# epam/Zstandard

Hardware: AMD Instinct MI355X
Metric: GiB/s compress @ level 3, 64 KiB chunks (higher is better)
Workload: dtype u8; 1 GPU; 4096 independent 65536 B chunks per GPU per step, level 3, BASELINE config[1] shape (Silesia unavailable offline -> Zipf-token log stream, SURVEY 8d); chunks_per_gpu=4096, chunk_bytes=65536, level=3, parallelism=chunks sharded over 1 GPU(s), no collective in the data path

## Files before the change

zstandard_amd/csrc/dict_train.hip:

```cpp
#include <hipcub/hipcub.hpp>
#include "zsmi_wave.h"
#include "entropy_kernels.hip"
#include "zsmi_fse.h"
#include "zsmi_status.h"
#include "zsmi_ctx.h"
#include <algorithm>

static const uint32_t kTrainDefaultF = 20, kTrainMinF = 12, kTrainMaxF = 26;
static const uint32_t kTrainDictSizeMin = 256, kTrainContentMin = 128;
static const uint32_t kTrainMaxZeroRun = 10;
static const uint32_t kTrainThreads = 1024, kTrainPerThread = 8;

struct ZsTrainCand { uint32_t k, d, pad0, pad1; uint32_t *freq; uint8_t *content; };

__device__ __forceinline__ uint32_t train_hash(const uint8_t *p, uint32_t d, uint32_t f)
{
    const uint64_t v = zs_load64(p);
    if (d == 6) return (uint32_t)(((v << 16) * 227718039650203ull) >> (64 - f));
    return (uint32_t)((v * 0xCF1BBCDCB7A56463ull) >> (64 - f));
}

__global__ void k_train_freq(const uint8_t *__restrict__ samples, uint32_t nbDmers, uint32_t d, uint32_t f, const uint64_t *__restrict__ ends, uint32_t nTrain,
                             uint2 *__restrict__ info, uint64_t *__restrict__ keys, uint32_t *__restrict__ freq)
{
// ... 112 lines not shown
        const uint32_t segSize = min(ne - nb + d - 1, tail);
        __syncthreads();
        if (segSize < d) break;
        tail -= segSize;
        for (uint32_t i = tid; i < segSize; i += kTrainThreads) content[tail + i] = samples[nb + i];
        __syncthreads();
    }
    if (tid == 0) tails[blockIdx.x] = tail;
}

__global__ void __launch_bounds__(64) k_train_id(const uint8_t *__restrict__ content, uint32_t size, uint32_t given, uint32_t *__restrict__ id)
{
    const uint64_t h = xxh64_quad<16>(content, size);
    if (threadIdx.x == 0) *id = given ? given : (uint32_t)(h % 2147450880ull) + 32768u;
}

__device__ static uint32_t train_scaled(const uint32_t *raw, uint32_t n, uint32_t *out, uint64_t limit)
{
    uint64_t total = 0;
    for (uint32_t s = 0; s < n; s++) total += (uint64_t)raw[s] + 1;
    uint32_t shift = 0;
    while ((total >> shift) >= limit) shift++;
    uint32_t sum = 0;
    for (uint32_t s = 0; s < n; s++) { out[s] = max(1u, (uint32_t)(((uint64_t)raw[s] + 1) >> shift)); sum += out[s]; }
    return sum;
}

__global__ void __launch_bounds__(256) k_train_tables(const uint32_t *__restrict__ stats, const uint8_t *__restrict__ content, uint32_t contentSize, uint32_t cap,
                                                      const uint32_t *__restrict__ dictID, uint8_t *__restrict__ hdr, uint8_t *__restrict__ out, uint32_t *__restrict__ result)
{
    __shared__ K3Lds L;
    __shared__ uint32_t cnt[64], misc[4];
    __shared__ int16_t norm[64];
    const uint32_t tid = threadIdx.x, wave = tid >> 6, lane = tid & 63u;
    const uint32_t hcap = 1024;
    if (tid == 0) { misc[0] = 0; misc[1] = 0; train_scaled(stats, 256, L.count, 1u << 23); }
    __syncthreads();
    const uint32_t lit = L.count[tid];
    for (uint32_t maxBits = ZS_HUF_MAXBITS; maxBits >= 8; maxBits--) {
        L.count[tid] = lit;
        __syncthreads();
        const uint32_t tableLog = huffLengths(L, 255, maxBits);
        huffCodesAndWeights(L, 255, tableLog);
        if (wave == 0) { const uint32_t hs = writeHuffHeaderWave(L, hdr + 8, 256, 255, tableLog); if (lane == 0) misc[0] = hs; }
        __syncthreads();
        if (misc[0]) break;
        __syncthreads();
    }
    if (wave == 0 && misc[0]) {
        uint32_t pos = 8 + misc[0];
        const uint32_t ofMax = zs_highbit(contentSize + (128u << 10));
        const uint32_t maxes[3] = { min(ofMax, (uint32_t)MaxOff), MaxML, MaxLL }, logs[3] = { OffFSELog, MLFSELog, LLFSELog }, base[3] = { 320, 384, 256 };
        bool ok = true;
        uint32_t &scaledTotal = L.misc[0], &ncountBytes = L.misc[1];
        for (uint32_t t = 0; t < 3 && ok; t++) {
            if (lane == 0) scaledTotal = train_scaled(stats + base[t], maxes[t] + 1, cnt, 1u << 30);
            wave_sync();
            normalizeCountsWave(norm, logs[t], cnt, scaledTotal, maxes[t]);
            if (lane == 0) ncountBytes = writeNCount(hdr + pos, hcap - pos, norm, maxes[t], logs[t]);
            wave_sync();
            const uint32_t w = ncountBytes;
            ok = w != 0; pos += w;
        }
        ok = ok && pos + 12 <= hcap;
        if (lane == 0) {
            const uint32_t id = *dictID, words[5] = { 0xEC30A437u, id, 1u, 4u, 8u };
            for (uint32_t i = 0; i < 2; i++) zs_store32(hdr + 4 * i, words[i]);
            if (ok) for (uint32_t i = 0; i < 3; i++) zs_store32(hdr + pos + 4 * i, words[2 + i]);
            pos += 12;
            misc[1] = (ok && pos <= hcap && pos < cap) ? pos : 0u;
        }
    }
    __syncthreads();
    const uint32_t hs = misc[1];
    if (!hs) { if (tid == 0) *result = 0; return; }
    const uint32_t keep = min(contentSize, cap - hs);
    for (uint32_t i = tid; i < hs; i += 256) out[i] = hdr[i];
    zs_block_copy(out + hs, content + (contentSize - keep), keep, tid, 256);
    if (tid == 0) *result = hs + keep;
}

__global__ void k_train_gather(const uint8_t *__restrict__ src, const uint64_t *__restrict__ offs , const uint32_t *__restrict__ sizes,
                               uint32_t n, uint8_t *__restrict__ dst)
{
    const uint32_t i = blockIdx.x;
    zs_block_copy(dst + offs[n + i], src + offs[i], sizes[i], threadIdx.x, blockDim.x);
}

extern "C" unsigned zsmi_getDictID(const void *dict, size_t dictSize)
{
    const uint8_t *d = (const uint8_t *)dict;
    if (!d || dictSize < 8 || rd32(d) != 0xEC30A437u) return 0;
    return rd32(d + 4);
}

namespace {
struct TrainPlan {
    uint32_t f = kTrainDefaultF, steps = 40;
    int level = 3;
    double split = 0.75;
    std::vector<std::pair<uint32_t, uint32_t>> cands;
    bool search = false;
};
}

static int trainParams(const zsmi_fastCoverParams *p, size_t cap, uint64_t total, uint32_t nb, TrainPlan &t)
{
    if (cap < kTrainDictSizeMin) return ZSMI_error_dstSize_tooSmall;
    if (!p) return ZSMI_error_GENERIC;
    if (p->d != 0 && p->d != 6 && p->d != 8) return ZSMI_error_parameter_outOfBound;
    if (p->f != 0 && (p->f < kTrainMinF || p->f > kTrainMaxF)) return ZSMI_error_parameter_outOfBound;
    if (p->accel > 1) return ZSMI_error_parameter_outOfBound;
    if (!(p->splitPoint == 0.0 || (p->splitPoint > 0.0 && p->splitPoint <= 1.0))) return ZSMI_error_parameter_outOfBound;
    if (p->k != 0 && (p->k < (p->d ? p->d : 8u) || p->k > cap || p->k > 65536u)) return ZSMI_error_parameter_outOfBound;
// ... 233 lines not shown
```

zstandard_amd/csrc/entropy_kernels.hip:

```cpp
#ifndef ZSMI_ENTROPY_KERNELS_HIP
#define ZSMI_ENTROPY_KERNELS_HIP
#include "zsmi_device.h"
#include "zsmi_status.h"
#include "zsmi_scratch.h"
#include "zsmi_wave.h"
#include "zsmi_fse.h"
#ifdef ZSMI_DEBUG_HOOKS
#define ZS_STOP_AT(v) (stopAt == (v))
#define ZS_STOPPED (stopAt != 0)
#else
#define ZS_STOP_AT(v) false
#define ZS_STOPPED false
#endif

__device__ __forceinline__ uint32_t llCodeOf(uint32_t ll)
{
    uint32_t c = zs_highbit(ll | 1u) + 19;
    c = (ll < 64) ? 24u : c;
    c = (ll < 48) ? 22u + ((ll - 32) >> 3) : c;
    c = (ll < 32) ? 20u + ((ll - 24) >> 2) : c;
    c = (ll < 24) ? 16u + ((ll - 16) >> 1) : c;
    return (ll < 16) ? ll : c;
}
__device__ __forceinline__ uint32_t mlCodeOf(uint32_t x)
{
    uint32_t c = zs_highbit(x | 1u) + 36;
    c = (x < 128) ? 42u : c;
    c = (x < 96) ? 40u + ((x - 64) >> 4) : c;
    c = (x < 64) ? 38u + ((x - 48) >> 3) : c;
    c = (x < 48) ? 36u + ((x - 40) >> 2) : c;
    c = (x < 40) ? 32u + ((x - 32) >> 1) : c;
    return (x < 32) ? x : c;
}
__device__ __forceinline__ uint32_t llExtraOf(uint32_t ll, uint32_t &bits)
{
    const uint32_t h = zs_highbit(ll | 1u);
    uint32_t v = ll - (1u << h), b = h;
    if (ll < 64) { v = ll - 48; b = 4; }
    if (ll < 48) { v = ll & 7u; b = 3; }
    if (ll < 32) { v = ll & 3u; b = 2; }
    if (ll < 24) { v = ll & 1u; b = 1; }
    if (ll < 16) { v = 0; b = 0; }
    bits = b; return v;
}
__device__ __forceinline__ uint32_t mlExtraOf(uint32_t x, uint32_t &bits)
{
    const uint32_t h = zs_highbit(x | 1u);
    uint32_t v = x - (1u << h), b = h;
    if (x < 128) { v = x - 96; b = 5; }
    if (x < 96) { v = x & 15u; b = 4; }
    if (x < 64) { v = x & 7u; b = 3; }
    if (x < 48) { v = x & 3u; b = 2; }
    if (x < 40) { v = x & 1u; b = 1; }
    if (x < 32) { v = 0; b = 0; }
    bits = b; return v;
}

struct FseCT {
    uint16_t stateTable[512];
    int32_t  deltaFindState[64];
    uint32_t deltaNbBits[64];
    uint32_t tableLog;
    uint32_t rle;
};
#define ZS_COST_NONE 0xFFFFu
struct ZsCDictTables {
    FseCT ct[3];
    uint16_t cost[3][64];
    uint32_t hufCodeNb[256];
    uint32_t hufLog;
};
__device__ __forceinline__ uint32_t fseSymbolCost(uint32_t nv, uint32_t tableLog)
{
    nv = max(nv, 1u);
    const uint32_t maxBitsOut = nv > 1 ? tableLog - zs_highbit(nv - 1) : tableLog;
    return maxBitsOut * 256u - ((((nv << maxBitsOut) - (1u << tableLog)) << 8) >> tableLog);
}
#ifndef ZS_LIT_MINWG
#define ZS_LIT_MINWG 8
#endif
struct K3Lds {
    uint32_t count[256];
    uint8_t  nbBits[256];
    uint32_t codeNb[256];
    uint32_t leafW[256];
    uint16_t leafSym[256];
    uint8_t  lenOfRank[256];
    uint8_t  weights[256];
    union {
        struct { uint32_t pkg[10][256]; uint32_t S[512]; uint32_t npk[12]; } pm;
        struct { FseCT ct; FseBuild build; uint16_t stepOut[256]; uint32_t bits[64]; } fse;
        struct { FseCT ct; FseBuild build; } cd[3];
        uint32_t tile[4][208];
        uint32_t hist[8][257];
        struct { uint32_t T[2052]; uint32_t wpar[4], wcnt[4]; uint32_t sel[16]; } gm;
    } u;
    uint32_t misc[16];
    uint32_t dictID;
    uint32_t wcount[16]; int16_t wnorm[16]; uint32_t rankStart[16], rankCount[16];
};
static_assert(sizeof(((K3Lds *)nullptr)->u.cd) <= offsetof(decltype(((K3Lds *)nullptr)->u.pm), S), "the digested dictionary's tables overlap the Huffman scratch S");
struct SeqLds {
    uint32_t count[192];
    FseCT ct[3];
    int16_t norm[64];
    union {
        FseBuild build;
        struct { uint32_t op[3][64]; } chain;
    } u;
    uint32_t tile[208];
    uint32_t misc[16];
};

struct BitSink {
    uint32_t *out32;
    uint32_t *tile;
    uint32_t bitpos;
};
__device__ __forceinline__ void sink_init(BitSink &b, void *out, uint32_t *tile)
{
    b.out32 = (uint32_t *)out; b.tile = tile; b.bitpos = 0;
    if (zs_lane() == 0) tile[0] = 0;
    wave_sync();
}
__device__ __forceinline__ void sink_put(BitSink &b, uint64_t lo, uint32_t hi, uint32_t nb)
{
    const uint32_t lane = (uint32_t)zs_lane();
    const uint32_t incl = wave_incl_scan(nb);
    const uint32_t total = wave_last(incl);
    const uint32_t base = b.bitpos & 31u;
    const uint32_t nwords = (base + total + 31u) >> 5;
    for (uint32_t i = 1 + lane; i <= nwords; i += 64) b.tile[i] = 0;
    wave_sync();
    if (nb) {
        const uint32_t bit = base + incl - nb;
        const uint32_t w = bit >> 5, sh = bit & 31u;
        const uint32_t v0 = (uint32_t)lo, v1 = (uint32_t)(lo >> 32), v2 = hi;
        const uint32_t w0 = v0 << sh;
        const uint32_t w1 = sh ? ((v1 << sh) | (v0 >> (32 - sh))) : v1;
        const uint32_t w2 = sh ? ((v2 << sh) | (v1 >> (32 - sh))) : v2;
        const uint32_t w3 = sh ? (v2 >> (32 - sh)) : 0u;
        if (w0) atomicOr(&b.tile[w], w0);
        if (w1) atomicOr(&b.tile[w + 1], w1);
        if (w2) atomicOr(&b.tile[w + 2], w2);
        if (w3) atomicOr(&b.tile[w + 3], w3);
    }
    wave_sync();
    const uint32_t nfull = (base + total) >> 5;
    uint32_t *dst = b.out32 + (b.bitpos >> 5);
    for (uint32_t i = lane; i < nfull; i += 64) dst[i] = b.tile[i];
    const uint32_t carry = b.tile[nfull];
    wave_sync();
    if (lane == 0) b.tile[0] = ((base + total) & 31u) ? carry : 0u;
    wave_sync();
    b.bitpos += total;
}
__device__ __forceinline__ uint32_t sink_close(BitSink &b)
{
    const uint32_t lane = (uint32_t)zs_lane();
    sink_put(b, lane == 0 ? 1ull : 0ull, 0u, lane == 0 ? 1u : 0u);
    if (lane == 0 && (b.bitpos & 31u)) b.out32[b.bitpos >> 5] = b.tile[0];
    wave_sync();
    return (b.bitpos + 7u) >> 3;
}

__device__ static uint32_t writeNCount(uint8_t *dst, uint32_t cap, const int16_t *norm, uint32_t maxSym, uint32_t tableLog)
{
    uint8_t *out = dst; uint8_t *const oend = dst + cap;
    const int tableSize = 1 << tableLog;
    int remaining = tableSize + 1, threshold = tableSize, nbBits = (int)tableLog + 1;
    uint32_t bitStream = 0; int bitCount = 0; uint32_t charnum = 0; int previous0 = 0;
    bitStream += (tableLog - 5) << bitCount; bitCount += 4;
    while (remaining > 1) {
        if (previous0) {
            uint32_t start = charnum;
            while (charnum <= maxSym && !norm[charnum]) charnum++;
            while (charnum >= start + 24) {
                start += 24; bitStream += 0xFFFFu << bitCount;
                if (out + 2 > oend) return 0;
                out[0] = (uint8_t)bitStream; out[1] = (uint8_t)(bitStream >> 8); out += 2; bitStream >>= 16;
            }
            while (charnum >= start + 3) { start += 3; bitStream += 3u << bitCount; bitCount += 2; }
            bitStream += (charnum - start) << bitCount; bitCount += 2;
            if (bitCount > 16) {
                if (out + 2 > oend) return 0;
                out[0] = (uint8_t)bitStream; out[1] = (uint8_t)(bitStream >> 8); out += 2; bitStream >>= 16; bitCount -= 16;
            }
        }
        {
            int count = norm[charnum++];
            const int max = (2 * threshold - 1) - remaining;
            remaining -= count < 0 ? -count : count;
            count++;
            if (count >= threshold) count += max;
            bitStream += (uint32_t)count << bitCount;
            bitCount += nbBits;
            bitCount -= (count < max);
            previous0 = (count == 1);
            while (remaining < threshold) { nbBits--; threshold >>= 1; }
        }
        if (bitCount > 16) {
            if (out + 2 > oend) return 0;
            out[0] = (uint8_t)bitStream; out[1] = (uint8_t)(bitStream >> 8); out += 2; bitStream >>= 16; bitCount -= 16;
        }
    }
    if (out + 2 > oend) return 0;
    out[0] = (uint8_t)bitStream; out[1] = (uint8_t)(bitStream >> 8);
    out += (bitCount + 7) / 8;
    return (uint32_t)(out - dst);
}

__device__ __forceinline__ void normalizeCountsWave(int16_t *norm, uint32_t tableLog, const uint32_t *count, uint32_t total, uint32_t maxSym)
{
    const uint32_t lane = (uint32_t)zs_lane();
    const uint32_t tableSize = 1u << tableLog;
    const uint32_t c = (lane <= maxSym) ? count[lane] : 0u;
    uint32_t p = 0;
    if (c) {
        const uint64_t scaled = (uint64_t)c * tableSize;
        p = (uint32_t)(scaled / total);
        const uint32_t rem = (uint32_t)(scaled % total);
        if (2 * (uint64_t)rem >= total) p++;
        if (p == 0) p = 1;
    }
    int still = (int)tableSize - (int)wave_sum(p);
    { const uint32_t key = (p << 6) | (63u - lane); const uint32_t best = wave_max(key); const uint32_t li = 63u - (best & 63u);
      if (still > 0 && lane == li) p += (uint32_t)still; }
    while (still < 0) {
        const uint32_t key = (p > 1) ? ((p << 6) | (63u - lane)) : 0u;
        const uint32_t best = wave_max(key);
        const uint32_t li = 63u - (best & 63u);
        if (lane == li) p--;
        still++;
    }
    if (lane <= maxSym) norm[lane] = (int16_t)p;
    wave_sync();
}

__device__ __forceinline__ void buildCTableWave(FseBuild &B, FseCT &ct, const int16_t *norm, uint32_t maxSym, uint32_t tableLog)
{
    const uint32_t lane = (uint32_t)zs_lane();
    const uint32_t tableSize = 1u << tableLog;
    const int n = (lane <= maxSym) ? (int)norm[lane] : 0;
    const uint32_t nv = n < 0 ? 1u : (uint32_t)n;
    const uint32_t excl = wave_incl_scan(nv) - nv;
    B.symCount[lane] = excl;
    if (lane <= maxSym) {
        if (nv == 0) { ct.deltaNbBits[lane] = ((tableLog + 1) << 16) - (1u << tableLog); ct.deltaFindState[lane] = 0; }
        else if (nv == 1) { ct.deltaNbBits[lane] = (tableLog << 16) - (1u << tableLog); ct.deltaFindState[lane] = (int)excl - 1; }
        else { const uint32_t maxBitsOut = tableLog - zs_highbit(nv - 1); ct.deltaNbBits[lane] = (maxBitsOut << 16) - (nv << maxBitsOut); ct.deltaFindState[lane] = (int)excl - (int)nv; }
    }
    if (lane == 0) { ct.tableLog = tableLog; ct.rle = 0; }
    fseSpreadWave(B.cumul, n, maxSym, tableLog, [&](uint32_t cell, uint32_t sym) __attribute__((always_inline)) { B.tableSymbol[cell] = (uint8_t)sym; });
    fseRankWave(B.symMask, B.symCount, tableSize, [&](uint32_t u) __attribute__((always_inline)) { return (uint32_t)B.tableSymbol[u]; },
                [&](uint32_t u, uint32_t, uint32_t next) __attribute__((always_inline)) { ct.stateTable[next] = (uint16_t)(tableSize + u); });
}
__device__ __forceinline__ uint32_t cstate_init(const FseCT &ct, uint32_t symbol)
{
    const uint32_t dnb = ct.deltaNbBits[symbol];
    const uint32_t nbBitsOut = (dnb + (1u << 15)) >> 16;
    const uint32_t v = (nbBitsOut << 16) - dnb;
    return ct.stateTable[(v >> nbBitsOut) + ct.deltaFindState[symbol]];
}

__device__ __forceinline__ uint32_t fseCompressWeightsWave(K3Lds &L, uint8_t *dst, uint32_t cap, const uint8_t *weights, uint32_t nw)
{
    const uint32_t lane = (uint32_t)zs_lane();
    if (lane == 0) {
        uint32_t tl = 0, maxSym = 0;
        do {
            const uint32_t *count = L.wcount;
            uint32_t tableLog;
            if (nw <= 1) break;
            for (uint32_t i = 0; i < 16; i++) if (count[i]) maxSym = i;
            bool one = false;
            for (uint32_t i = 0; i <= maxSym; i++) if (count[i] == nw) one = true;
            if (one) break;
            tableLog = 6;
            while (tableLog > 5 && (1u << (tableLog - 1)) >= nw) tableLog--;
            { uint32_t present = 0; for (uint32_t i = 0; i <= maxSym; i++) present += count[i] != 0; if (present > (1u << tableLog)) break; }
            tl = tableLog;
        } while (0);
        L.misc[13] = tl; L.misc[14] = maxSym;
    }
    L.u.fse.bits[lane] = 0;
    wave_sync();
    const uint32_t tableLog = L.misc[13], maxSym = L.misc[14];
    if (!tableLog) return 0;
    normalizeCountsWave(L.wnorm, tableLog, L.wcount, nw, maxSym);
    if (lane == 0) L.misc[12] = writeNCount(dst, cap, L.wnorm, maxSym, tableLog);
    wave_sync();
    const uint32_t hsize = L.misc[12];
    if (!hsize) return 0;
    buildCTableWave(L.u.fse.build, L.u.fse.ct, L.wnorm, maxSym, tableLog);
    const FseCT &ct = L.u.fse.ct;
    const uint32_t K = nw - 2;
    uint16_t *stepOut = L.u.fse.stepOut;
    uint32_t fin = 0;
    if (lane < 2) {
        uint32_t st = cstate_init(ct, weights[nw - 1 - lane]);
        for (uint32_t k = lane; k < K; k += 2) {
            const uint32_t sym = weights[nw - 3 - k];
            const uint32_t nbo = (st + ct.deltaNbBits[sym]) >> 16;
            stepOut[k] = (uint16_t)((st & ((1u << nbo) - 1u)) | (nbo << 8));
            st = ct.stateTable[(st >> nbo) + ct.deltaFindState[sym]];
        }
        fin = st;
    }
    wave_sync();
    const uint32_t stFirst = wave_get(fin, 0), stSecond = wave_get(fin, 1);
    const uint32_t st2 = (nw & 1u) ? stSecond : stFirst, st1 = (nw & 1u) ? stFirst : stSecond;
    uint32_t *bits = L.u.fse.bits;
    uint32_t total = 0;
    for (uint32_t k0 = 0; k0 < K + 3; k0 += 64) {
        const uint32_t k = k0 + lane;
        uint32_t val = 0, nb = 0;
        if (k < K) { const uint32_t e = stepOut[k]; val = e & 0xFFu; nb = e >> 8; }
        else if (k == K) { val = st2 & ((1u << tableLog) - 1u); nb = tableLog; }
        else if (k == K + 1) { val = st1 & ((1u << tableLog) - 1u); nb = tableLog; }
        else if (k == K + 2) { val = 1; nb = 1; }
        const uint32_t incl = wave_incl_scan(nb);
        const uint32_t off = total + incl - nb;
        if (nb) {
            const uint32_t w = off >> 5, sh = off & 31u;
            atomicOr(&bits[w], val << sh);
            if (sh + nb > 32u) atomicOr(&bits[w + 1], val >> (32u - sh));
        }
        total += wave_last(incl);
    }
    wave_sync();
    const uint32_t bytes = (total + 7u) >> 3;
    if (bytes > cap - hsize) return 0;
    const uint8_t *bb = reinterpret_cast<const uint8_t *>(bits);
    for (uint32_t j = lane; j < bytes; j += 64) dst[hsize + j] = bb[j];
    return hsize + bytes;
}

__device__ __forceinline__ uint32_t writeHuffHeaderWave(K3Lds &L, uint8_t *dst, uint32_t cap, uint32_t maxSym, uint32_t tableLog)
{
    const uint32_t lane = (uint32_t)zs_lane();
    uint8_t *weights = L.weights;
    if (maxSym >= 2 && cap > 1) {
        const uint32_t h = fseCompressWeightsWave(L, dst + 1, cap - 1 < 127 ? cap - 1 : 127, weights, maxSym);
        if (h > 1 && h < maxSym / 2 && h < 128) { if (lane == 0) dst[0] = (uint8_t)h; return h + 1; }
    }
    if (maxSym > 128) return 0;
    if ((maxSym + 1) / 2 + 1 > cap) return 0;
    if (lane == 0) { dst[0] = (uint8_t)(128 + (maxSym - 1)); weights[maxSym] = 0; }
    wave_sync();
    for (uint32_t s = 2 * lane; s < maxSym; s += 128) dst[s / 2 + 1] = (uint8_t)((weights[s] << 4) + weights[s + 1]);
    return (maxSym + 1) / 2 + 1;
}

__device__ static uint32_t lowerBound(const uint32_t *a, uint32_t n, uint32_t key)
{ uint32_t lo = 0, hi = n; while (lo < hi) { const uint32_t mid = (lo + hi) >> 1; if (a[mid] < key) lo = mid + 1; else hi = mid; } return lo; }
__device__ static uint32_t upperBound(const uint32_t *a, uint32_t n, uint32_t key)
{ uint32_t lo = 0, hi = n; while (lo < hi) { const uint32_t mid = (lo + hi) >> 1; if (a[mid] <= key) lo = mid + 1; else hi = mid; } return lo; }

__device__ static uint32_t huffLengths(K3Lds &L, uint32_t maxSym, uint32_t maxBits)
{
    const uint32_t tid = threadIdx.x;
    const uint32_t c = (tid <= maxSym) ? L.count[tid] : 0u;
    L.nbBits[tid] = 0;
    uint32_t *keys = L.u.pm.S;
    const uint32_t lane_ = tid & 63u, wave_ = tid >> 6;
    const uint64_t pres = __ballot(c != 0);
    if (lane_ == 0) L.u.pm.npk[4 + wave_] = (uint32_t)__popcll(pres);
    __syncthreads();
    uint32_t before = 0, n = 0;
    #pragma unroll
    for (uint32_t v = 0; v < 4; v++) { const uint32_t k = L.u.pm.npk[4 + v]; if (v < wave_) before += k; n += k; }
    const uint32_t key = (c << 8) | tid;
    if (c) keys[before + (uint32_t)__popcll(pres & ((1ull << lane_) - 1ull))] = key;
    __syncthreads();
    if (c) {
        uint32_t rank = 0;
        for (uint32_t t = 0; t < n; t++) rank += (keys[t] < key) ? 1u : 0u;
        L.leafW[rank] = c; L.leafSym[rank] = (uint16_t)tid;
    }
    __syncthreads();
    if (n == 1) { if (tid == 0) L.nbBits[L.leafSym[0]] = 1; __syncthreads(); return 1; }
    uint32_t (*pkg)[256] = L.u.pm.pkg;
    uint32_t *S = L.u.pm.S;
    uint32_t *npk = L.u.pm.npk;
    if (tid == 0) npk[1] = 0;
    __syncthreads();
    for (uint32_t level = 2; level <= maxBits; level++) {
        const uint32_t np = npk[level - 1];
        const uint32_t *prev = (level >= 3) ? pkg[level - 3] : nullptr;
        if (tid < n) { const uint32_t w = L.leafW[tid]; S[tid + (np ? lowerBound(prev, np, w) : 0u)] = w; }
        if (tid < np) { const uint32_t w = prev[tid]; S[tid + upperBound(L.leafW, n, w)] = w; }
        __syncthreads();
        const uint32_t have = (n + np) >> 1;
        if (tid < have) pkg[level - 2][tid] = S[2 * tid] + S[2 * tid + 1];
        if (tid == 0) npk[level] = have;
        __syncthreads();
    }
    L.lenOfRank[tid] = 0;
    __syncthreads();
    uint32_t m = 2 * n - 2;
    for (uint32_t level = maxBits; level >= 1; level--) {
        const uint32_t np = npk[level];
        const uint32_t *cur = (level >= 2) ? pkg[level - 2] : nullptr;
        if (m > n + np) m = n + np;
        bool in = false;
        if (tid < n) { const uint32_t pos = tid + (np ? lowerBound(cur, np, L.leafW[tid]) : 0u); in = pos < m; }
        const uint32_t li = (uint32_t)__syncthreads_count(in);
        if (in) L.lenOfRank[tid]++;
        const uint32_t pi = m - li;
        m = 2 * pi;
        if (!m) break;
    }
    __syncthreads();
    if (tid < n) L.nbBits[L.leafSym[tid]] = L.lenOfRank[tid];
    __syncthreads();
    return L.lenOfRank[0];
}

__device__ static void huffCodesAndWeights(K3Lds &L, uint32_t maxSym, uint32_t tableLog)
{
    const uint32_t tid = threadIdx.x, lane = tid & 63u, wave = tid >> 6;
    const uint32_t nb = (tid <= maxSym) ? L.nbBits[tid] : 0u;
    const uint32_t w = nb ? tableLog + 1 - nb : 0u;
    if (tid < 16) { L.rankCount[tid] = 0; L.wcount[tid] = 0; }
    __syncthreads();
    if (nb) atomicAdd(&L.rankCount[w], 1u);
    if (tid < maxSym) { L.weights[tid] = (uint8_t)w; atomicAdd(&L.wcount[w], 1u); }
    __syncthreads();
    if (tid == 0) { uint32_t next = 0; for (uint32_t k = 1; k <= tableLog; k++) { L.rankStart[k] = next; next += L.rankCount[k] << (k - 1); } }
    uint32_t idx = 0;
    for (uint32_t k = 1; k <= tableLog; k++) {
        const uint64_t m = __ballot(w == k);
        if (w == k) idx = (uint32_t)__popcll(m & ((1ull << lane) - 1));
        if (lane == 0) L.u.pm.S[wave * 16 + k] = (uint32_t)__popcll(m);
    }
    __syncthreads();
    if (nb) {
        for (uint32_t v = 0; v < wave; v++) idx += L.u.pm.S[v * 16 + w];
        L.codeNb[tid] = ((L.rankStart[w] >> (w - 1)) + idx) | (nb << 16);
    }
    __syncthreads();
}

__device__ __forceinline__ uint32_t huffEncodeStream(K3Lds &L, uint32_t *tile, uint8_t *tmp, const uint8_t *lits, uint32_t from, uint32_t len)
{
    const uint32_t lane = (uint32_t)zs_lane();
    BitSink sink; sink_init(sink, tmp, tile);
    uint32_t remaining = len;
    const uint32_t k0 = lane * 8;
    auto fetch = [&](uint32_t rem) -> uint64_t {
        const uint32_t T = min(512u, rem);
        uint64_t e = 0;
        if (k0 + 8 <= T) e = zs_load64(lits + from + rem - 8 - k0);
        else for (uint32_t j = 0; j < 8; j++) if (k0 + j < T) e |= (uint64_t)lits[from + rem - 1 - k0 - j] << (8 * (7 - j));
        return e;
    };
    uint64_t next = remaining ? fetch(remaining) : 0ull;
    while (remaining) {
        const uint32_t T = min(512u, remaining);
        const uint64_t eight = next;
        if (remaining > T) next = fetch(remaining - T);
        uint32_t cn[8];
        #pragma unroll
        for (uint32_t j = 0; j < 8; j++) cn[j] = L.codeNb[(uint32_t)(eight >> (8 * (7 - j))) & 0xFFu];
        #pragma unroll
        for (uint32_t j = 0; j < 8; j++) cn[j] = (k0 + j < T) ? cn[j] : 0u;
        uint32_t pv[4], pn[4];
        #pragma unroll
        for (uint32_t j = 0; j < 4; j++) {
            const uint32_t b0 = cn[2 * j] >> 16;
            pv[j] = (cn[2 * j] & 0xFFFFu) | ((cn[2 * j + 1] & 0xFFFFu) << b0);
            pn[j] = b0 + (cn[2 * j + 1] >> 16);
        }
        const uint64_t q0 = (uint64_t)pv[0] | ((uint64_t)pv[1] << pn[0]), q1 = (uint64_t)pv[2] | ((uint64_t)pv[3] << pn[2]);
        const uint32_t n0 = pn[0] + pn[1];
        const uint64_t lo = q0 | (q1 << n0);
        const uint32_t hi = (uint32_t)((q1 >> 1) >> (63u - n0));
        const uint32_t nb = n0 + pn[2] + pn[3];
        sink_put(sink, lo, hi, nb);
        remaining -= T;
    }
    return sink_close(sink);
}

__device__ __forceinline__ int lastFlagBelow(bool flag)
{
    const uint64_t m = __ballot(flag);
    const uint32_t lane = (uint32_t)zs_lane();
    const uint64_t below = lane ? (m & ((1ull << lane) - 1)) : 0ull;
    return below ? 63 - __builtin_clzll(below) : -1;
}

struct ZsChunkDesc { uint64_t srcOff; uint64_t dstOff; uint32_t size; uint32_t firstBlock; uint32_t nBlocks; uint32_t pad; };
// ... 530 lines not shown
        }
        wave_sync();
        if (ZS_STOP_AT(1)) break;

        uint32_t pos = hdrBytes + 1;
        uint32_t modeByte = 0;
        bool fail = false;
        auto repeatBeats = [&](uint32_t t, uint32_t c, uint32_t est) -> bool {
            const uint32_t dc = cdt->cost[t][lane];
            if (__any(c != 0 && dc == ZS_COST_NONE)) return false;
            if (wave_sum(c * dc) >= est) return false;
            const uint32_t *from = reinterpret_cast<const uint32_t *>(&cdt->ct[t]); uint32_t *to = reinterpret_cast<uint32_t *>(&L.ct[t]);
            for (uint32_t i = lane; i < sizeof(FseCT) / 4; i += 64) to[i] = from[i];
            return true;
        };
        #pragma unroll 1
        for (uint32_t t = 0; t < 3; t++) {
            const uint32_t *count = L.count + 64 * t;
            const uint32_t maxCode = t == 0 ? MaxLL : (t == 1 ? MaxOff : MaxML);
            const uint32_t maxLog = t == 0 ? LLFSELog : (t == 1 ? OffFSELog : MLFSELog);
            const uint32_t defLog = t == 0 ? LL_defaultNormLog : (t == 1 ? OF_defaultNormLog : ML_defaultNormLog), defMax = t == 0 ? MaxLL : (t == 1 ? DefaultMaxOff : MaxML);
            FseCT &ct = L.ct[t];
            const uint32_t c = (lane <= maxCode) ? count[lane] : 0u;
            const uint64_t present = __ballot(c != 0);
            const uint32_t maxSym = 63u - (uint32_t)__builtin_clzll(present);
            const uint32_t largest = wave_max(c);
            uint32_t mode;
            if (largest == nseq) {
                mode = 1;
                if (pos >= cap) { fail = true; break; }
                if constexpr (CD) { if (cdt && repeatBeats(t, c, 8u * 256u)) mode = 3; }
                if (mode == 1) {
                if (lane == 0) { out[pos] = (uint8_t)maxSym; ct.rle = 1; ct.tableLog = 0; }
                pos += 1;
                }
            } else if (nseq < 64 && maxSym <= defMax) {
                mode = 0;
                if constexpr (CD) {
                    if (cdt) {
                        const int16_t *defNorm = t == 0 ? LL_defaultNorm : (t == 1 ? OF_defaultNorm : ML_defaultNorm);
                        const int nv = lane <= defMax ? defNorm[lane] : 1;
                        if (repeatBeats(t, c, wave_sum(c * fseSymbolCost((uint32_t)(nv < 0 ? 1 : nv), defLog)))) mode = 3;
                    }
                }
                if (mode == 0) buildCTableWave(L.u.build, ct, t == 0 ? LL_defaultNorm : (t == 1 ? OF_defaultNorm : ML_defaultNorm), defMax, defLog);
            } else {
                uint32_t tableLog = maxLog;
                { const uint32_t hb = zs_highbit(nseq - 1); const uint32_t want = hb > 2 ? hb - 2 : 5; if (want < tableLog) tableLog = want; }
                { const uint32_t minBits = zs_highbit(maxSym) + 2; const uint32_t npresent = (uint32_t)__popcll(present);
                  if (tableLog < minBits) tableLog = minBits; while ((1u << tableLog) < npresent) tableLog++; }
                if (tableLog < 5) tableLog = 5;
                if (tableLog > maxLog) tableLog = maxLog;
                normalizeCountsWave(L.norm, tableLog, count, nseq, maxSym);
                if (lane == 0) L.misc[0] = writeNCount(out + pos, cap - pos, L.norm, maxSym, tableLog);
                wave_sync();
                const uint32_t h = L.misc[0];
                if (!h) { fail = true; break; }
                mode = 2;
                if constexpr (CD) {
                    if (cdt && repeatBeats(t, c, h * 8u * 256u + wave_sum(c ? c * fseSymbolCost((uint32_t)L.norm[lane], tableLog) : 0u))) mode = 3;
                }
                if (mode == 2) {
                pos += h;
                buildCTableWave(L.u.build, ct, L.norm, maxSym, tableLog);
                }
            }
            modeByte |= mode << (6 - 2 * t);
            wave_sync();
        }
        if (fail) break;
        if (ZS_STOP_AT(2)) break;
        if (lane == 0) out[hdrBytes] = (uint8_t)modeByte;
        bitstreamOff = pos;
        live = true;
    } while (0);

    uint8_t *bsTmp = out + ((bitstreamOff + 3u) & ~3u);
    BitSink sink; sink_init(sink, bsTmp, L.tile);
    const uint32_t bsCap = ZS_SEQSEC_STRIDE - ((bitstreamOff + 3u) & ~3u) - 1024u;
    bool overflow = false;
    if (live && !ZS_STOP_AT(3)) {
        const uint32_t nFull = nseq >> 4, tail = nseq & 15u;
        uint32_t Sb = max((nFull + ZS_CHAIN_MAXSEG - 1u) / ZS_CHAIN_MAXSEG, (uint32_t)ZS_CHAIN_MINSEG);
        const uint32_t K = max((nFull + Sb - 1u) / Sb, 1u);
        const uint32_t c = (lane >= K ? 1u : 0u) + (lane >= 2u * K ? 1u : 0u), k = lane - c * K;
        const bool chainLane = lane < 3u * K && !L.ct[min(c, 2u)].rle;
        const FseCT &ct = L.ct[min(c, 2u)];
        const uint8_t *codes = chainCodes + (size_t)min(c, 2u) * ZS_CHAIN_CODES;
        uint16_t *outs = chainOuts + (size_t)min(c, 2u) * ZS_CHAIN_CODES;
        typedef const __attribute__((address_space(3))) uint16_t *LdsU16;
        typedef const __attribute__((address_space(3))) uint32_t *LdsU32;
        #pragma unroll
        for (uint32_t t = 0; t < 3; t++) L.u.chain.op[t][lane] = L.ct[t].deltaNbBits[lane] | ((uint32_t)(L.ct[t].deltaFindState[lane] + 1024) << 20);
        wave_sync();
        const uint32_t tabAddr = (uint32_t)(uintptr_t)(LdsU16)ct.stateTable - 2048u, opAddr = (uint32_t)(uintptr_t)(LdsU32)L.u.chain.op[min(c, 2u)];
        const uint32_t firstOut = k * Sb, bEnd = min(firstOut + Sb, nFull);
        const bool lastSeg = k + 1u == K;
        const uint32_t bWarm = firstOut > ZS_CHAIN_WARM / 16u ? firstOut - ZS_CHAIN_WARM / 16u : 0u;
        #define CHAIN_STEP(sym, o) { \
            const uint32_t op_ = *(LdsU32)(uintptr_t)(opAddr + ((sym) << 2)); \
            const uint32_t nbo_ = __builtin_amdgcn_ubfe(state + op_, 16, 4); \
            (o) = __builtin_amdgcn_ubfe(state, 0, nbo_) | (nbo_ << 12); \
            state = *(LdsU16)(uintptr_t)(tabAddr + (((state >> nbo_) + (op_ >> 20)) << 1)); }
        typedef uint32_t u32x4 __attribute__((ext_vector_type(4)));
        uint8_t *junk = zs_seqsec_lend_junk_store(out, lane);
        auto runBlocks = [&](uint32_t from, uint32_t to, uint32_t outFrom, uint32_t mark, uint32_t &state, uint32_t &entry, uint32_t rounds) {
            u32x4 cw;
            {
                const uint8_t *a0 = codes + 16u * min(from, nFull ? nFull - 1u : 0u);
// ... 334 lines not shown
```

Before: 152.4 GiB/s.

## Parallelize FSE NCount header writing across the wave with scans

Replaces the serial lane-0 writeNCount loop with a wave-parallel version. Each lane computes its symbol's bit piece from a prefix scan of remaining cells and a zero-run ballot, then ORs it into an LDS bit buffer with atomics and copies the bytes out. It also adds a 32-bit division fast path to normalizeCountsWave, keeping the 64-bit path for dictionary training. The aim is to cut the serial latency of table-header emission in the sequence-compression path, at the cost of LDS atomics and more exact reliance on matching the reference bit format.

New measurement: 152.7 GiB/s, median of 5. Within noise of the previous version (+0.2%).

```diff
diff --git a/zstandard_amd/csrc/dict_train.hip b/zstandard_amd/csrc/dict_train.hip
--- a/zstandard_amd/csrc/dict_train.hip
+++ b/zstandard_amd/csrc/dict_train.hip
@@ -188,14 +188,12 @@
         const uint32_t ofMax = zs_highbit(contentSize + (128u << 10));
         const uint32_t maxes[3] = { min(ofMax, (uint32_t)MaxOff), MaxML, MaxLL }, logs[3] = { OffFSELog, MLFSELog, LLFSELog }, base[3] = { 320, 384, 256 };
         bool ok = true;
-        uint32_t &scaledTotal = L.misc[0], &ncountBytes = L.misc[1];
+        uint32_t &scaledTotal = L.misc[0];
         for (uint32_t t = 0; t < 3 && ok; t++) {
             if (lane == 0) scaledTotal = train_scaled(stats + base[t], maxes[t] + 1, cnt, 1u << 30);
             wave_sync();
-            normalizeCountsWave(norm, logs[t], cnt, scaledTotal, maxes[t]);
-            if (lane == 0) ncountBytes = writeNCount(hdr + pos, hcap - pos, norm, maxes[t], logs[t]);
-            wave_sync();
-            const uint32_t w = ncountBytes;
+            normalizeCountsWave<true>(norm, logs[t], cnt, scaledTotal, maxes[t]);
+            const uint32_t w = writeNCountWave(hdr + pos, hcap - pos, norm, maxes[t], logs[t], L.u.tile[0]);
             ok = w != 0; pos += w;
         }
         ok = ok && pos + 12 <= hcap;
diff --git a/zstandard_amd/csrc/entropy_kernels.hip b/zstandard_amd/csrc/entropy_kernels.hip
--- a/zstandard_amd/csrc/entropy_kernels.hip
+++ b/zstandard_amd/csrc/entropy_kernels.hip
@@ -5,6 +5,7 @@
 #include "zsmi_scratch.h"
 #include "zsmi_wave.h"
 #include "zsmi_fse.h"
+#include "zsmi_ncount.h"
 #ifdef ZSMI_DEBUG_HOOKS
 #define ZS_STOP_AT(v) (stopAt == (v))
 #define ZS_STOPPED (stopAt != 0)
@@ -164,52 +165,32 @@
     return (b.bitpos + 7u) >> 3;
 }
 
-__device__ static uint32_t writeNCount(uint8_t *dst, uint32_t cap, const int16_t *norm, uint32_t maxSym, uint32_t tableLog)
-{
-    uint8_t *out = dst; uint8_t *const oend = dst + cap;
-    const int tableSize = 1 << tableLog;
-    int remaining = tableSize + 1, threshold = tableSize, nbBits = (int)tableLog + 1;
-    uint32_t bitStream = 0; int bitCount = 0; uint32_t charnum = 0; int previous0 = 0;
-    bitStream += (tableLog - 5) << bitCount; bitCount += 4;
-    while (remaining > 1) {
-        if (previous0) {
-            uint32_t start = charnum;
-            while (charnum <= maxSym && !norm[charnum]) charnum++;
-            while (charnum >= start + 24) {
-                start += 24; bitStream += 0xFFFFu << bitCount;
-                if (out + 2 > oend) return 0;
-                out[0] = (uint8_t)bitStream; out[1] = (uint8_t)(bitStream >> 8); out += 2; bitStream >>= 16;
-            }
-            while (charnum >= start + 3) { start += 3; bitStream += 3u << bitCount; bitCount += 2; }
-            bitStream += (charnum - start) << bitCount; bitCount += 2;
-            if (bitCount > 16) {
-                if (out + 2 > oend) return 0;
-                out[0] = (uint8_t)bitStream; out[1] = (uint8_t)(bitStream >> 8); out += 2; bitStream >>= 16; bitCount -= 16;
-            }
-        }
-        {
-            int count = norm[charnum++];
-            const int max = (2 * threshold - 1) - remaining;
-            remaining -= count < 0 ? -count : count;
-            count++;
-            if (count >= threshold) count += max;
-            bitStream += (uint32_t)count << bitCount;
-            bitCount += nbBits;
-            bitCount -= (count < max);
-            previous0 = (count == 1);
-            while (remaining < threshold) { nbBits--; threshold >>= 1; }
-        }
-        if (bitCount > 16) {
-            if (out + 2 > oend) return 0;
-            out[0] = (uint8_t)bitStream; out[1] = (uint8_t)(bitStream >> 8); out += 2; bitStream >>= 16; bitCount -= 16;
-        }
-    }
-    if (out + 2 > oend) return 0;
-    out[0] = (uint8_t)bitStream; out[1] = (uint8_t)(bitStream >> 8);
-    out += (bitCount + 7) / 8;
-    return (uint32_t)(out - dst);
-}
-
+__device__ __forceinline__ uint32_t writeNCountWave(uint8_t *dst, uint32_t cap, const int16_t *norm, uint32_t maxSym, uint32_t tableLog, uint32_t *bits)
+{
+    const uint32_t lane = (uint32_t)zs_lane();
+    const int n = (lane <= maxSym) ? (int)norm[lane] : 0;
+    const int nPrev = (int)ZS_DPP(0, n, 0x138, 0xF, true);
+    const uint32_t cells = (uint32_t)(n < 0 ? -n : n);
+    const int remaining = (int)((1u << tableLog) + 1u) - (int)(wave_incl_scan(cells) - cells);
+    const uint64_t zeros = __ballot(lane <= maxSym && n == 0);
+    const uint32_t zerosBehind = (uint32_t)__builtin_ctzll(((~zeros >> lane) >> 1) | (1ull << 63));
+    const ZsNCountPiece p = zs_ncount_piece(lane, maxSym, n, nPrev, zerosBehind, remaining, tableLog);
+    const uint32_t incl = wave_incl_scan(p.width);
+    const uint32_t total = wave_last(incl);
+    if (zs_ncount_refused(total, cap)) return 0;
+    #pragma unroll 1
+    for (uint32_t i = lane; i < (total + 31u) >> 5; i += 64) bits[i] = 0;
+    wave_sync();
+    zs_ncount_place(p.value, incl - p.width, [&](uint32_t i, uint32_t v) __attribute__((always_inline)) { atomicOr(&bits[i], v); });
+    wave_sync();
+    const uint8_t *bb = reinterpret_cast<const uint8_t *>(bits);
+    #pragma unroll 1
+    for (uint32_t j = lane; j < zs_ncount_touched(total); j += 64) dst[j] = bb[j];
+    wave_sync();
+    return zs_ncount_size(total);
+}
+
+template <bool WIDE = false>
 __device__ __forceinline__ void normalizeCountsWave(int16_t *norm, uint32_t tableLog, const uint32_t *count, uint32_t total, uint32_t maxSym)
 {
     const uint32_t lane = (uint32_t)zs_lane();
@@ -217,10 +198,16 @@
     const uint32_t c = (lane <= maxSym) ? count[lane] : 0u;
     uint32_t p = 0;
     if (c) {
-        const uint64_t scaled = (uint64_t)c * tableSize;
-        p = (uint32_t)(scaled / total);
-        const uint32_t rem = (uint32_t)(scaled % total);
-        if (2 * (uint64_t)rem >= total) p++;
+        if constexpr (WIDE) {
+            const uint64_t scaled = (uint64_t)c * tableSize;
+            p = (uint32_t)(scaled / total);
+            const uint32_t rem = (uint32_t)(scaled % total);
+            if (2 * (uint64_t)rem >= total) p++;
+        } else {
+            const uint32_t scaled = c << tableLog;
+            p = scaled / total;
+            if (2 * (scaled - p * total) >= total) p++;
+        }
         if (p == 0) p = 1;
     }
     int still = (int)tableSize - (int)wave_sum(p);
@@ -283,15 +270,13 @@
         } while (0);
         L.misc[13] = tl; L.misc[14] = maxSym;
     }
-    L.u.fse.bits[lane] = 0;
     wave_sync();
     const uint32_t tableLog = L.misc[13], maxSym = L.misc[14];
     if (!tableLog) return 0;
     normalizeCountsWave(L.wnorm, tableLog, L.wcount, nw, maxSym);
-    if (lane == 0) L.misc[12] = writeNCount(dst, cap, L.wnorm, maxSym, tableLog);
-    wave_sync();
-    const uint32_t hsize = L.misc[12];
+    const uint32_t hsize = writeNCountWave(dst, cap, L.wnorm, maxSym, tableLog, L.u.fse.bits);
     if (!hsize) return 0;
+    L.u.fse.bits[lane] = 0;
     buildCTableWave(L.u.fse.build, L.u.fse.ct, L.wnorm, maxSym, tableLog);
     const FseCT &ct = L.u.fse.ct;
     const uint32_t K = nw - 2;
@@ -1075,9 +1060,7 @@
                 if (tableLog < 5) tableLog = 5;
                 if (tableLog > maxLog) tableLog = maxLog;
                 normalizeCountsWave(L.norm, tableLog, count, nseq, maxSym);
-                if (lane == 0) L.misc[0] = writeNCount(out + pos, cap - pos, L.norm, maxSym, tableLog);
-                wave_sync();
-                const uint32_t h = L.misc[0];
+                const uint32_t h = writeNCountWave(out + pos, cap - pos, L.norm, maxSym, tableLog, L.tile);
                 if (!h) { fail = true; break; }
                 mode = 2;
                 if constexpr (CD) {
diff --git a/zstandard_amd/csrc/zsmi_ncount.h b/zstandard_amd/csrc/zsmi_ncount.h
--- /dev/null
+++ b/zstandard_amd/csrc/zsmi_ncount.h
@@ -0,0 +1,45 @@
+#pragma once
+#include <stdint.h>
+#if defined(__HIPCC__)
+#define ZS_NCOUNT_FN __host__ __device__ __forceinline__
+#else
+#define ZS_NCOUNT_FN static inline
+#endif
+
+struct ZsNCountPiece { uint64_t value; uint32_t width; };
+ZS_NCOUNT_FN ZsNCountPiece zs_ncount_piece(uint32_t s, uint32_t maxSym, int n, int nPrev, uint32_t zerosBehind, int remaining, uint32_t tableLog)
+{
+    ZsNCountPiece p;
+    p.value = 0; p.width = 0;
+    if (s == 0) { p.value = tableLog - 5; p.width = 4; }
+    if (s > maxSym || remaining <= 1 || (s > 0 && n == 0 && nPrev == 0)) return p;
+    const uint32_t hb = 31u - (uint32_t)__builtin_clz((uint32_t)remaining);
+    const int threshold = 1 << hb, max = 2 * threshold - 1 - remaining;
+    int count = n + 1;
+    if (count >= threshold) count += max;
+    p.value |= (uint64_t)(uint32_t)count << p.width;
+    p.width += hb + 1 - (count < max ? 1u : 0u);
+    if (n == 0) {
+        uint32_t r = zerosBehind;
+        const uint32_t esc = r / 24; r -= 24 * esc;
+        const uint32_t threes = r / 3; r -= 3 * threes;
+        p.value |= ((1ull << (16 * esc)) - 1) << p.width; p.width += 16 * esc;
+        p.value |= ((1ull << (2 * threes)) - 1) << p.width; p.width += 2 * threes;
+        p.value |= (uint64_t)r << p.width; p.width += 2;
+    }
+    return p;
+}
+ZS_NCOUNT_FN uint32_t zs_ncount_size(uint32_t totalBits) { return (totalBits + 7u) >> 3; }
+ZS_NCOUNT_FN uint32_t zs_ncount_touched(uint32_t totalBits) { return 2u * ((totalBits + 15u) >> 4); }
+ZS_NCOUNT_FN bool zs_ncount_refused(uint32_t totalBits, uint32_t cap) { return zs_ncount_touched(totalBits) > cap; }
+template <class OrWord>
+ZS_NCOUNT_FN void zs_ncount_place(uint64_t value, uint32_t bit, OrWord &&orWord)
+{
+    const uint32_t w = bit >> 5, sh = bit & 31u, lo = (uint32_t)value, hi = (uint32_t)(value >> 32);
+    const uint32_t w0 = lo << sh;
+    const uint32_t w1 = sh ? ((hi << sh) | (lo >> (32u - sh))) : hi;
+    const uint32_t w2 = sh ? (hi >> (32u - sh)) : 0u;
+    if (w0) orWord(w, w0);
+    if (w1) orWord(w + 1, w1);
+    if (w2) orWord(w + 2, w2);
+}
```

## Restructure package-merge Huffman length build to cut barriers and binary searches

Applied to the files above, without the earlier changes.

Replaces the binary-search merge and the per-level barrier-counted backward pass in the Huffman length builder. The new version uses padded, branch-free fixed-step searches, caches placement offsets packed into bytes, and computes per-level inclusion with wave ballots and closed-form package counts. Code and weight assignment drops the atomics and serial rank-start loop in favour of ballots, a cross-wave table and a wave scan. The aim is to remove __syncthreads and serial work in the literal Huffman stage. The cost is more complex indexing that depends on MAXBITS==11 and on n<=256.

Measured after the change: 151.2 GiB/s before, 152.9 GiB/s after, median of 6. +1.1%, better.

```diff
diff --git a/zstandard_amd/csrc/entropy_kernels.hip b/zstandard_amd/csrc/entropy_kernels.hip
--- a/zstandard_amd/csrc/entropy_kernels.hip
+++ b/zstandard_amd/csrc/entropy_kernels.hip
@@ -85,10 +85,9 @@
     uint32_t codeNb[256];
     uint32_t leafW[256];
     uint16_t leafSym[256];
-    uint8_t  lenOfRank[256];
     uint8_t  weights[256];
     union {
-        struct { uint32_t pkg[10][256]; uint32_t S[512]; uint32_t npk[12]; } pm;
+        struct { uint32_t pkg[10][256]; uint32_t S[512]; } pm;
         struct { FseCT ct; FseBuild build; uint16_t stepOut[256]; uint32_t bits[64]; } fse;
         struct { FseCT ct; FseBuild build; } cd[3];
         uint32_t tile[4][208];
@@ -97,7 +96,7 @@
     } u;
     uint32_t misc[16];
     uint32_t dictID;
-    uint32_t wcount[16]; int16_t wnorm[16]; uint32_t rankStart[16], rankCount[16];
+    uint32_t wcount[16]; int16_t wnorm[16];
 };
 static_assert(sizeof(((K3Lds *)nullptr)->u.cd) <= offsetof(decltype(((K3Lds *)nullptr)->u.pm), S), "the digested dictionary's tables overlap the Huffman scratch S");
 struct SeqLds {
@@ -352,24 +351,46 @@
     return (maxSym + 1) / 2 + 1;
 }
 
-__device__ static uint32_t lowerBound(const uint32_t *a, uint32_t n, uint32_t key)
-{ uint32_t lo = 0, hi = n; while (lo < hi) { const uint32_t mid = (lo + hi) >> 1; if (a[mid] < key) lo = mid + 1; else hi = mid; } return lo; }
-__device__ static uint32_t upperBound(const uint32_t *a, uint32_t n, uint32_t key)
-{ uint32_t lo = 0, hi = n; while (lo < hi) { const uint32_t mid = (lo + hi) >> 1; if (a[mid] <= key) lo = mid + 1; else hi = mid; } return lo; }
+#define ZS_PM_PAD 0xFFFFFFFFu
+__device__ __forceinline__ void pmSearch(const uint32_t *pk, uint32_t w, uint32_t &lb, const uint32_t *lf, uint32_t pw, uint32_t &ub, bool wide)
+{
+    uint32_t a = 0, b = 0;
+    if (wide) {
+        uint32_t ca = 0, cb = 0;
+        #pragma unroll
+        for (uint32_t j = 1; j < 4; j++) { ca += pk[64 * j - 1] < w; cb += lf[64 * j - 1] <= pw; }
+        a = 64 * ca; b = 64 * cb;
+    }
+    {
+        uint32_t ca = 0, cb = 0;
+        #pragma unroll
+        for (uint32_t j = 1; j < 8; j++) { ca += pk[a + 8 * j - 1] < w; cb += lf[b + 8 * j - 1] <= pw; }
+        a += 8 * ca; b += 8 * cb;
+    }
+    {
+        uint32_t ca = 0, cb = 0;
+        #pragma unroll
+        for (uint32_t j = 0; j < 8; j++) { ca += pk[a + j] < w; cb += lf[b + j] <= pw; }
+        a += ca; b += cb;
+    }
+    lb = a; ub = b;
+}
+__device__ __forceinline__ uint32_t pmPackages(uint32_t n, uint32_t level) { return (n * ((1u << (level - 1)) - 1u)) >> (level - 1); }
 
 __device__ static uint32_t huffLengths(K3Lds &L, uint32_t maxSym, uint32_t maxBits)
 {
+    static_assert(ZS_HUF_MAXBITS == 11, "K3Lds::u.pm.pkg and the place bytes are laid out for levels 2..11");
     const uint32_t tid = threadIdx.x;
     const uint32_t c = (tid <= maxSym) ? L.count[tid] : 0u;
     L.nbBits[tid] = 0;
     uint32_t *keys = L.u.pm.S;
     const uint32_t lane_ = tid & 63u, wave_ = tid >> 6;
     const uint64_t pres = __ballot(c != 0);
-    if (lane_ == 0) L.u.pm.npk[4 + wave_] = (uint32_t)__popcll(pres);
+    if (lane_ == 0) L.misc[12 + wave_] = (uint32_t)__popcll(pres);
     __syncthreads();
     uint32_t before = 0, n = 0;
     #pragma unroll
-    for (uint32_t v = 0; v < 4; v++) { const uint32_t k = L.u.pm.npk[4 + v]; if (v < wave_) before += k; n += k; }
+    for (uint32_t v = 0; v < 4; v++) { const uint32_t k = L.misc[12 + v]; if (v < wave_) before += k; n += k; }
     const uint32_t key = (c << 8) | tid;
     if (c) keys[before + (uint32_t)__popcll(pres & ((1ull << lane_) - 1ull))] = key;
     __syncthreads();
@@ -378,43 +399,64 @@
         for (uint32_t t = 0; t < n; t++) rank += (keys[t] < key) ? 1u : 0u;
         L.leafW[rank] = c; L.leafSym[rank] = (uint16_t)tid;
     }
+    if (tid >= n) L.leafW[tid] = ZS_PM_PAD;
     __syncthreads();
     if (n == 1) { if (tid == 0) L.nbBits[L.leafSym[0]] = 1; __syncthreads(); return 1; }
     uint32_t (*pkg)[256] = L.u.pm.pkg;
     uint32_t *S = L.u.pm.S;
-    uint32_t *npk = L.u.pm.npk;
-    if (tid == 0) npk[1] = 0;
-    __syncthreads();
-    for (uint32_t level = 2; level <= maxBits; level++) {
-        const uint32_t np = npk[level - 1];
-        const uint32_t *prev = (level >= 3) ? pkg[level - 3] : nullptr;
-        if (tid < n) { const uint32_t w = L.leafW[tid]; S[tid + (np ? lowerBound(prev, np, w) : 0u)] = w; }
-        if (tid < np) { const uint32_t w = prev[tid]; S[tid + upperBound(L.leafW, n, w)] = w; }
+    const uint32_t w = L.leafW[tid];
+    uint32_t np = n >> 1;
+    uint32_t pw = tid < np ? L.leafW[2 * tid] + L.leafW[2 * tid + 1] : ZS_PM_PAD;
+    pkg[0][tid] = pw;
+    uint32_t lbs[3];
+    lbs[0] = lbs[1] = lbs[2] = tid < n ? 0u : 0xFFFFFFFFu;
+    __syncthreads();
+    #pragma unroll 1
+    for (uint32_t level = 3; level <= maxBits + 1; level++) {
+        uint32_t lb = 0, ub = 0;
+        if (64 * wave_ < n) pmSearch(pkg[level - 3], w, lb, L.leafW, pw, ub, n > 64);
+        if (tid < n) {
+            const uint32_t q = level - 3, sh = 8 * (q & 3);
+            #pragma unroll
+            for (uint32_t k = 0; k < 3; k++) lbs[k] |= (q >> 2) == k ? lb << sh : 0u;
+        }
+        if (level > maxBits) break;
+        if (tid < n) S[tid + lb] = w;
+        if (tid < np) S[tid + ub] = pw;
         __syncthreads();
-        const uint32_t have = (n + np) >> 1;
-        if (tid < have) pkg[level - 2][tid] = S[2 * tid] + S[2 * tid + 1];
-        if (tid == 0) npk[level] = have;
+        np = (n + np) >> 1;
+        pw = tid < np ? S[2 * tid] + S[2 * tid + 1] : ZS_PM_PAD;
+        pkg[level - 2][tid] = pw;
         __syncthreads();
     }
-    L.lenOfRank[tid] = 0;
-    __syncthreads();
-    uint32_t m = 2 * n - 2;
-    for (uint32_t level = maxBits; level >= 1; level--) {
-        const uint32_t np = npk[level];
-        const uint32_t *cur = (level >= 2) ? pkg[level - 2] : nullptr;
-        if (m > n + np) m = n + np;
-        bool in = false;
-        if (tid < n) { const uint32_t pos = tid + (np ? lowerBound(cur, np, L.leafW[tid]) : 0u); in = pos < m; }
-        const uint32_t li = (uint32_t)__syncthreads_count(in);
-        if (in) L.lenOfRank[tid]++;
-        const uint32_t pi = m - li;
-        m = 2 * pi;
-        if (!m) break;
-    }
-    __syncthreads();
-    if (tid < n) L.nbBits[L.leafSym[tid]] = L.lenOfRank[tid];
-    __syncthreads();
-    return L.lenOfRank[0];
+    uint32_t (*place)[256] = pkg;
+    #pragma unroll
+    for (uint32_t k = 0; k < 3; k++) place[k][tid] = lbs[k];
+    __syncthreads();
+    uint32_t pl[4][3];
+    #pragma unroll
+    for (uint32_t j = 0; j < 4; j++) {
+        #pragma unroll
+        for (uint32_t k = 0; k < 3; k++) pl[j][k] = place[k][lane_ + 64 * j];
+    }
+    uint32_t m = 2 * n - 2, mine = 0, longest = 0;
+    #pragma unroll
+    for (uint32_t level = ZS_HUF_MAXBITS; level >= 1; level--) {
+        if (level > maxBits) continue;
+        m = min(m, n + pmPackages(n, level));
+        uint32_t li = 0;
+        #pragma unroll
+        for (uint32_t j = 0; j < 4; j++) {
+            const uint32_t lb = level >= 2 ? (pl[j][(level - 2) >> 2] >> (8 * ((level - 2) & 3))) & 0xFFu : 0u;
+            li += (uint32_t)__popcll(__ballot(lane_ + 64 * j + lb < m));
+        }
+        mine += tid < li;
+        longest += li != 0;
+        m = 2 * (m - li);
+    }
+    if (tid < n) L.nbBits[L.leafSym[tid]] = (uint8_t)mine;
+    __syncthreads();
+    return longest;
 }
 
 __device__ static void huffCodesAndWeights(K3Lds &L, uint32_t maxSym, uint32_t tableLog)
@@ -422,23 +464,28 @@
     const uint32_t tid = threadIdx.x, lane = tid & 63u, wave = tid >> 6;
     const uint32_t nb = (tid <= maxSym) ? L.nbBits[tid] : 0u;
     const uint32_t w = nb ? tableLog + 1 - nb : 0u;
-    if (tid < 16) { L.rankCount[tid] = 0; L.wcount[tid] = 0; }
-    __syncthreads();
-    if (nb) atomicAdd(&L.rankCount[w], 1u);
-    if (tid < maxSym) { L.weights[tid] = (uint8_t)w; atomicAdd(&L.wcount[w], 1u); }
-    __syncthreads();
-    if (tid == 0) { uint32_t next = 0; for (uint32_t k = 1; k <= tableLog; k++) { L.rankStart[k] = next; next += L.rankCount[k] << (k - 1); } }
-    uint32_t idx = 0;
+    if (tid < maxSym) L.weights[tid] = (uint8_t)w;
+    uint32_t idx = 0, cnt = 0, last = 0;
+    {
+        const uint64_t m = __ballot(w == 0 && tid < maxSym);
+        if (lane == 0) cnt = (uint32_t)__popcll(m);
+    }
     for (uint32_t k = 1; k <= tableLog; k++) {
         const uint64_t m = __ballot(w == k);
         if (w == k) idx = (uint32_t)__popcll(m & ((1ull << lane) - 1));
-        if (lane == 0) L.u.pm.S[wave * 16 + k] = (uint32_t)__popcll(m);
-    }
-    __syncthreads();
-    if (nb) {
-        for (uint32_t v = 0; v < wave; v++) idx += L.u.pm.S[v * 16 + w];
-        L.codeNb[tid] = ((L.rankStart[w] >> (w - 1)) + idx) | (nb << 16);
-    }
+        if (lane == k) { cnt = (uint32_t)__popcll(m); last = (uint32_t)((m >> (maxSym & 63u)) & 1u); }
+    }
+    if (lane < 16) L.u.pm.S[wave * 16 + lane] = cnt | (wave == (maxSym >> 6) ? last << 16 : 0u);
+    __syncthreads();
+    uint32_t tot = 0, lower = 0, isLast = 0;
+    #pragma unroll
+    for (uint32_t v = 0; v < 4; v++) { const uint32_t x = L.u.pm.S[v * 16 + (lane & 15u)]; tot += x & 0xFFFFu; if (v < wave) lower += x & 0xFFFFu; isLast |= x >> 16; }
+    const uint32_t k_ = lane & 15u;
+    const uint32_t cells = (k_ >= 1 && k_ <= tableLog) ? tot << (k_ - 1) : 0u;
+    const uint32_t start = wave_incl_scan(cells) - cells;
+    if (tid < 16) L.wcount[tid] = k_ <= tableLog ? tot - isLast : 0u;
+    const uint32_t rs = (uint32_t)__shfl((int)start, (int)w), lw = (uint32_t)__shfl((int)lower, (int)w);
+    if (nb) L.codeNb[tid] = ((rs >> (w - 1)) + lw + idx) | (nb << 16);
     __syncthreads();
 }
 
```
